# OER-9000/MB-iSTFT-VITS

Hardware: AMD Instinct MI355X
Metric: audio samples/sec (22.05 kHz), MB-iSTFT-VITS infer, batch 64 per GPU (higher is better)
Workload: dtype f32; 1 GPU; configs[1]: ljs_mb_istft_vits, batch 64 per GPU, infer(noise_scale=0, length_scale=1), all 8 outputs; global_batch=64, t_text=200, t_frames_max=566, parallelism=utterance-sharded dp1

## Files before the change

include/mbistft_vits.h:

```cpp
#ifndef MBISTFT_VITS_H
#define MBISTFT_VITS_H

#include <stddef.h>
#include <stdint.h>

#ifdef __cplusplus
extern "C" {
#endif

#define MBV_ABI_VERSION 3

#define MBV_DEC_MULTIBAND   0
#define MBV_DEC_MULTISTREAM 1
#define MBV_DEC_SINGLEBAND  2

typedef struct mbv_model mbv_model;

typedef struct mbv_config {
  int32_t struct_bytes;
  int32_t n_vocab;
  int32_t inter_channels;
  int32_t hidden_channels;
  int32_t filter_channels;
  int32_t n_heads;
// ... 200 lines not shown
  const float *chan_add;
  const float *res;
  const float *res_chan_add;
  const float *accum_in;
  float out_scale;
  const int64_t *trim_lens;
  int32_t trim_num, trim_add;
  int32_t splitk;
  int32_t prec;
  int32_t legacy_convt;
  int64_t ws_floats;
  int32_t n_counters;
  const float *ln_gamma;
  const float *ln_beta;
  const int32_t *ln_out_lens;
} mbv_conv_desc;
#define MBV_ROUTE_NARROW_M 1
#define MBV_ROUTE_NARROW_LAUNCH 2
#define MBV_ROUTE_M64 3
#define MBV_ROUTE_HALF 4
#define MBV_ROUTE_SMALL 5
#define MBV_ROUTE_BIG 6
#define MBV_ROUTE_SPLIT_BATCH 7
#define MBV_ROUTE_VS 8
int mbv_op_conv(mbv_model *m, const mbv_conv_desc *d, const float *x, const float *w_host, const float *bias_host,
                float *y, int32_t *plan_out, void *stream);
int mbv_conv_plan(const mbv_conv_desc *d, int32_t out[8]);

int mbv_op_embed(mbv_model *m, const int64_t *ids, const int64_t *lengths, const float *emb, float *x, int32_t *lens32,
                 int32_t *bad, int B, int T, int H, int n_vocab, void *stream);
int mbv_op_layernorm(mbv_model *m, const float *a, const float *r, const float *gamma, const float *beta, float *y,
                     int B, int C, int T, int pre_relu, const int32_t *out_lens, void *stream);
int mbv_op_durations(mbv_model *m, const float *h, const float *w, const float *bias, const int32_t *lens,
                     float length_scale, float *logw, float *w_ceil, int32_t *cum, int32_t *ylen32, int64_t *ylen64,
                     const int32_t *bad, int B, int C, int T, void *stream);
int mbv_op_expand(mbv_model *m, const float *stats, const int32_t *cum, const int32_t *ylen32, const float *noise,
                  float noise_scale, float *m_p, float *logs_p, float *z_p, float *z, float *attn, float *y_mask,
                  int B, int I, int T, int Tp, void *stream);
int mbv_op_cond_gemv(mbv_model *m, const float *g, const float *W, const float *bias, float *out, int B, int Cin,
                     int Cout, void *stream);
int mbv_op_gather_rows(mbv_model *m, const float *table, const int64_t *sid, float *out, int B, int C, int n_rows,
                       int32_t *bad, void *stream);
// ... 26 lines not shown
```

mb-istft-vits_amd/_capi.py:

```python
import ctypes as C
import os
import subprocess

_HERE = os.path.dirname(os.path.abspath(__file__))
CSRC = os.path.join(_HERE, "csrc")
LIB_PATH = os.environ.get("MBV_LIB") or os.path.join(CSRC, "libmbistft_vits.so")

SYMBOLS = [
    "mbv_abi_version", "mbv_create", "mbv_destroy", "mbv_last_error", "mbv_load_weight",
    "mbv_finalize_weights", "mbv_missing_weights", "mbv_encode", "mbv_synthesize", "mbv_decode",
    "mbv_speaker_embedding", "mbv_stage_times_ms", "mbv_istft_pqmf", "mbv_read_stage",
    "mbv_op_conv1d", "mbv_kernel_times_ms", "mbv_istft_finalize", "mbv_pcm16", "mbv_voice_conversion",
    "mbv_set_option", "mbv_arena_floats", "mbv_export_arena", "mbv_import_arena", "mbv_ticket", "mbv_stage_times_ms_at", "mbv_op_rel_attention",
    "mbv_pcm16_samples", "mbv_resample", "mbv_resample_bank", "mbv_op_conv", "mbv_conv_plan",
    "mbv_spectrogram", "mbv_spectrogram_frames", "mbv_decoder_context", "mbv_decode_range",
    "mbv_resample_ready", "mbv_resample_pcm16_range",
    "mbv_ragged_classes", "mbv_decode_ragged", "mbv_synthesize_ragged", "mbv_ragged_plan",
    "mbv_chunks_plan", "mbv_decode_chunks", "mbv_decoder_runs",
    "mbv_pcm_chunks_plan", "mbv_resample_pcm16_chunks", "mbv_wire_runs",
    "mbv_op_embed", "mbv_op_layernorm", "mbv_op_durations", "mbv_op_expand", "mbv_op_cond_gemv", "mbv_op_gather_rows",
    "mbv_op_posterior_sample", "mbv_op_lens", "mbv_op_dds_sep", "mbv_op_dds_res", "mbv_op_sdp_pre", "mbv_op_sdp_spline",
    "mbv_op_sdp_logw", "mbv_op_sdp_noise", "mbv_op_chan_add",
    "mbv_align", "mbv_set_durations", "mbv_op_neg_cent", "mbv_op_max_path",
    "mbv_admit_plan", "mbv_encode_rows", "mbv_synthesize_rows", "mbv_encoder_runs", "mbv_get_option",
]


ABI_VERSION = 3

# ... 40 lines not shown

class MbvAlignOutputs(C.Structure):
    _fields_ = [(n, C.c_void_p) for n in
                ("w", "attn", "x_mask", "y_mask", "z", "z_p", "m_p", "logs_p", "neg_cent")]


class MbvConvDesc(C.Structure):
    _fields_ = [(n, C.c_int32) for n in ("B", "Cin", "Cout", "Tin", "T", "K", "dil", "x_rstride", "kind", "epi")] + [
        ("in_slope", C.c_float), ("relu", C.c_int32), ("reflect1", C.c_int32),
        ("in_lens", C.c_void_p), ("out_lens", C.c_void_p), ("chan_add", C.c_void_p), ("res", C.c_void_p),
        ("res_chan_add", C.c_void_p), ("accum_in", C.c_void_p), ("out_scale", C.c_float),
        ("trim_lens", C.c_void_p), ("trim_num", C.c_int32), ("trim_add", C.c_int32),
        ("splitk", C.c_int32), ("prec", C.c_int32), ("legacy_convt", C.c_int32),
        ("ws_floats", C.c_int64), ("n_counters", C.c_int32),
        ("ln_gamma", C.c_void_p), ("ln_beta", C.c_void_p), ("ln_out_lens", C.c_void_p),
    ]


CONV_KIND_CONV, CONV_KIND_CONVT4, CONV_KIND_CONVT8 = 0, 4, 8
CONV_EPI_STORE, CONV_EPI_RESID, CONV_EPI_RESID_ACC, CONV_EPI_LN = 0, 1, 2, 7
ROUTES = {1: "NARROW_M", 2: "NARROW_LAUNCH", 3: "M64", 4: "HALF", 5: "SMALL", 6: "BIG", 7: "SPLIT_BATCH", 8: "VS"}
PLAN_FIELDS = ("route", "bm", "bn", "threads", "ck", "nb_big", "vs_tv", "S")


def build(force=False, verbose=False):
    if force:
        for f in os.listdir(CSRC):
            if f.endswith(".o") or f.endswith(".so"):
                os.remove(os.path.join(CSRC, f))
    r = subprocess.run(["bash", os.path.join(CSRC, "build.sh")], capture_output=True, text=True)
# ... 51 lines not shown
    L.mbv_spectrogram_frames.restype = C.c_int64
    L.mbv_set_option.argtypes = [vp, C.c_char_p, i32]
    L.mbv_ticket.argtypes = [vp]
    L.mbv_ticket.restype = C.c_int64
    L.mbv_stage_times_ms_at.argtypes = [vp, C.c_int64, C.POINTER(C.c_float * 5)]
    L.mbv_arena_floats.argtypes = [vp]
    L.mbv_arena_floats.restype = C.c_int64
    L.mbv_export_arena.argtypes = [vp, vp, C.c_int64, vp]
    L.mbv_import_arena.argtypes = [vp, vp, C.c_int64, vp]
    L.mbv_read_stage.argtypes = [vp, C.c_char_p, vp, C.c_int64, vp]
    L.mbv_read_stage.restype = C.c_int64
    L.mbv_op_rel_attention.argtypes = [vp, vp, vp, vp, vp, vp, i32, i32, i32, i32, vp]
    L.mbv_op_conv1d.argtypes = [vp, vp, vp, vp, vp, i32, i32, i32, i32, i32, i32, C.c_float, vp]
    L.mbv_op_conv.argtypes = [vp, C.POINTER(MbvConvDesc), vp, vp, vp, vp, C.POINTER(C.c_int32 * 8), vp]
    L.mbv_conv_plan.argtypes = [C.POINTER(MbvConvDesc), C.POINTER(C.c_int32 * 8)]
    f32 = C.c_float
    L.mbv_op_embed.argtypes = [vp, vp, vp, vp, vp, vp, vp, i32, i32, i32, i32, vp]
    L.mbv_op_layernorm.argtypes = [vp, vp, vp, vp, vp, vp, i32, i32, i32, i32, vp, vp]
    L.mbv_op_durations.argtypes = [vp, vp, vp, vp, vp, f32, vp, vp, vp, vp, vp, vp, i32, i32, i32, vp]
    L.mbv_op_expand.argtypes = [vp, vp, vp, vp, vp, f32, vp, vp, vp, vp, vp, vp, i32, i32, i32, i32, vp]
    L.mbv_op_cond_gemv.argtypes = [vp, vp, vp, vp, vp, i32, i32, i32, vp]
    L.mbv_op_gather_rows.argtypes = [vp, vp, vp, vp, i32, i32, i32, vp, vp]
    L.mbv_op_posterior_sample.argtypes = [vp, vp, vp, vp, vp, i32, i32, i32, vp]
    L.mbv_op_lens.argtypes = [vp, vp, vp, vp, vp, i32, i32, vp]
    L.mbv_op_dds_sep.argtypes = [vp, vp, vp, vp, vp, vp, vp, vp, i32, i32, i32, i32, i32, vp]
    L.mbv_op_dds_res.argtypes = [vp, vp, vp, vp, vp, vp, i32, i32, i32, vp, vp]
    L.mbv_op_sdp_pre.argtypes = [vp, vp, i32, vp, vp, vp, vp, i32, i32, i32, vp]
    L.mbv_op_sdp_spline.argtypes = [vp, vp, vp, vp, i32, i32, i32, f32, vp]
    L.mbv_op_sdp_logw.argtypes = [vp, vp, vp, vp, vp, vp, i32, i32, vp]
    L.mbv_op_sdp_noise.argtypes = [vp, vp, f32, vp, C.c_int64, vp]
# ... 51 lines not shown
```

mb-istft-vits_amd/csrc/capi.hip:

```cpp
#include "../../include/mbistft_vits.h"
#include "kernels.h"

#include <algorithm>
#include <array>
#include <cmath>
#include <cstdarg>
#include <cstdio>
#include <cstdlib>
#include <cstring>
#include <map>
#include <string>
#include <vector>

using namespace mbv;

namespace {

constexpr int kWindow = 4;
constexpr int kDpFilter = 256;
constexpr int kFlowLayers = 4;
constexpr int kFlowK = 5;
constexpr int kNFlows = 4;
constexpr float kLrelu = 0.1f;

// ... 1052 lines not shown
            a.accum_in = j == 0 ? nullptr : xs;
            a.out_scale = j == 2 ? (1.f / 3.f) : 1.f;
          }
          if (rr) a.in_lens = i == 0 ? rr->len_u : rr->len_uu;
          with_trim(a, Lo / Td, 0);
          launch_conv1d(a, s, rt_num * (Lo / Td));
          state = r;
        }
        continue;
      }
      for (int q = 0; q < 3; ++q) {
        const int d = c.resblock_dilations[j][q];
        {
          ConvArgs a = conv_args(m, R.c1[q], state, (int64_t)ch * Lo, Lo, t1, (int64_t)ch * Lo, Lo, B, d);
          a.in_slope = kLrelu;
          if (q == 0) a.chan_add = cadd;
          own_ws(a);
          if (rr) a.in_lens = i == 0 ? rr->len_u : rr->len_uu;
          with_trim(a, Lo / Td, 0);
          launch_conv1d(a, s, rt_num * (Lo / Td));
        }
        {
          ConvArgs a = conv_args(m, R.c2[q], t1, (int64_t)ch * Lo, Lo, r, (int64_t)ch * Lo, Lo, B, 1);
          a.in_slope = kLrelu;
          a.res = state; a.res_bstride = (int64_t)ch * Lo;
          if (q == 0) a.res_chan_add = cadd;
          if (q < 2) {
            a.epi = EPI_RESID;
          } else {
            a.epi = EPI_RESID_ACC;
            a.y = xs;
            a.accum_in = j == 0 ? nullptr : xs;
            a.out_scale = j == 2 ? (1.f / 3.f) : 1.f;
            if (conc && j > 0) HIPCHK(m, hipStreamWaitEvent(s, m->ev_rb[j - 1], 0));
          }
          own_ws(a);
          if (rr) a.in_lens = i == 0 ? rr->len_u : rr->len_uu;
          with_trim(a, Lo / Td, 0);
          launch_conv1d(a, s, rt_num * (Lo / Td));
// ... 2247 lines not shown
  }
  ConvArgs a{};
  a.Tin = d.Tin; a.x_rstride = d.x_rstride ? d.x_rstride : d.Tin; a.Cin = d.Cin;
  a.x_bstride = (int64_t)d.Cin * a.x_rstride;
  a.M = convt ? U * d.Cout : d.Cout;
  a.Mpad = (int)align_up(a.M, 128);
  a.K = convt ? 16 / U + 1 : d.K;
  a.dil = convt ? 1 : d.dil;
  a.pad_left = convt ? (U == 4 ? 2 : 1) : (a.K - 1) * a.dil / 2;
  a.in_slope = d.in_slope;
  a.in_lens = d.in_lens; a.chan_add = d.chan_add; a.reflect1 = d.reflect1;
  a.T = d.T;
  a.y_bstride = (int64_t)d.Cout * d.T * (convt ? U : 1);
  a.epi = convt ? EPI_CONVT : d.epi;
  a.convt_u = convt ? U : 0;
  a.relu = d.relu; a.out_lens = d.out_lens;
  a.res = d.res; a.res_bstride = (int64_t)d.Cout * d.T; a.res_chan_add = d.res_chan_add;
  a.accum_in = d.accum_in; a.out_scale = d.epi == MBV_CONV_EPI_RESID_ACC ? d.out_scale : 1.f;
  a.B = d.B;
  a.splitk = d.splitk != 0;
  a.prec = d.prec;
  if ((a.epi == EPI_RESID || a.epi == EPI_RESID_ACC) && (unsigned long long)a.M * a.T * 4ull >= (1ull << 32))
    return "one utterance's output exceeds 4 GiB";
  if (ln) {
    a.ln_gamma = d.ln_gamma; a.ln_beta = d.ln_beta; a.ln_out_lens = d.ln_out_lens;
    if (!conv1d_narrow_supported(a)) return "LN outside the narrow kernel's range (conv1d_narrow_supported)";
  }
  *out = a;
  return nullptr;
}

// ... 25 lines not shown
int mbv_conv_plan(const mbv_conv_desc* d, int32_t out[8]) {
  if (!d || !out) { g_create_error = "mbv_conv_plan: NULL argument"; return 1; }
  ConvArgs a{};
  const char* why = conv_desc_args(*d, &a);
  ConvPlan p{};
  if (!why) {
    a.ws_floats = d->ws_floats > 0 ? (size_t)d->ws_floats : 0;
    a.n_counters = d->n_counters > 0 ? d->n_counters : 0;
    why = conv_desc_plan(*d, a, &p);
  }
  if (why) { g_create_error = std::string("mbv_conv_plan: ") + why; return 1; }
  plan_ints(p, out);
  return 0;
}

int mbv_op_conv(mbv_model* m, const mbv_conv_desc* d, const float* x, const float* w_host, const float* bias_host,
                float* y, int32_t* plan_out, void* stream) {
  if (!m) return 1;
  if (!d || !x || !w_host || !y) return m->fail("mbv_op_conv: NULL argument");
  ConvArgs a{};
  const char* why = conv_desc_args(*d, &a);
  if (why) return m->fail("mbv_op_conv: %s", why);
  a.ws = m->conv_ws; a.ws_floats = m->conv_ws_floats; a.counters = m->conv_cnt; a.n_counters = m->conv_ncnt;
  if (m->splitk && !d->trim_lens) a.splitk = 1;
  ConvPlan p{};
  if ((why = conv_desc_plan(*d, a, &p))) return m->fail("mbv_op_conv: %s", why);
  DEVICE_GUARD(m);
  hipStream_t s = (hipStream_t)stream;
  DevAllocs mem;
  auto upload = [&](const void* src, size_t bytes, void** dst) -> int {
    HIPCHK(m, hipMalloc(dst, bytes));
    mem.p.push_back(*dst);
    HIPCHK(m, hipMemcpy(*dst, src, bytes, hipMemcpyHostToDevice));
    return 0;
  };
  const bool convt = a.epi == EPI_CONVT;
  const int U = a.convt_u;
// ... 45 lines not shown
```

mb-istft-vits_amd/csrc/conv1d.hip:

```cpp
#include "kernels.h"
#include <cstdio>
#include <cstdlib>

#ifndef MBV_CONV_GLDS
#define MBV_CONV_GLDS 8
#endif
namespace mbv {

typedef float f32x16 __attribute__((ext_vector_type(16)));
typedef float f32x4 __attribute__((ext_vector_type(4)));

__device__ __forceinline__ float lrelu(float v, float slope) { return v > 0.f ? v : v * slope; }
__device__ __forceinline__ float sigmoidf_(float v) { return 1.f / (1.f + expf(-v)); }

#ifdef MBV_CONV_STAMPS
#define MBV_CSTAMP(ID)                                                                        \
  if ((tid & 255) == 0 && stamp_n < 511) stamp_lds[tid >> 8][++stamp_n] = (__builtin_amdgcn_s_memrealtime() << 4) | (unsigned)(ID);
#define MBV_CSTAMP_FLUSH()                                                                    \
  {                                                                                           \
    if ((tid & 255) == 0) stamp_lds[tid >> 8][0] = stamp_n;                                   \
    __syncthreads();                                                                          \
    unsigned long long* sb_ = reinterpret_cast<unsigned long long*>(a.ws) + (size_t)blockIdx.x * 1024; \
    for (int e = tid; e < 1024; e += NT) sb_[e] = stamp_lds[e >> 9][e & 511];                 \
  }
// ... 117 lines not shown
                if (a.accum_in) v0 += a.accum_in[(int64_t)b * a.y_bstride + (int64_t)row * a.T + t];
              } else if constexpr (EPI == EPI_RES_SKIP) {
                if (row < a.split) v0 = a.y[(int64_t)b * a.y_bstride + (int64_t)row * a.T + t];
                else if (a.skip_accum) v0 = a.skip[((int64_t)b * (a.M - a.split) + (row - a.split)) * a.T + t];
              } else {
                v0 = a.couple_sign * a.y[(int64_t)b * a.y_bstride + (int64_t)row * a.T + t];
              }
            }
          }
          acc[i][j][r] = v0;
        }
      }
    }
}

template <int WM, int WN, int CK, int NWN, int EPI, int PREC = 0, int NWM = 2, int VS = 0>
__global__ __launch_bounds__(64 * NWM * NWN, 2) void conv1d_mfma_kernel(const ConvArgs a, int tiles_x,
                                                                        int tiles_y, int total_tiles,
                                                                        int ksplit) {
  constexpr int NT = 64 * NWM * NWN;
  constexpr bool DB = NWN == 4;
  constexpr int BM = 32 * WM * NWM;
  constexpr int BN = 32 * WN * NWN;
  constexpr int G = CK / 8;
  extern __shared__ __attribute__((aligned(16))) float lds[];

  const int tid = threadIdx.x;
  const int lane = tid & 63;
#ifdef MBV_CONV_STAMPS
  int stamp_n = 0;
  __shared__ unsigned long long stamp_lds[2][512];
// ... 5 lines not shown
  const int halo = (a.K - 1) * a.dil;
  const int XL = BN + halo;
  const int buf_f4 = G * 2 * XL + a.K * G * 2 * BM + 2 * BM;
  f32x4* const lds4 = reinterpret_cast<f32x4*>(lds);
  const int tin_eff = a.reflect1 ? a.Tin + 1 : a.Tin;

  constexpr int HALO_MAX = CK == 8 ? 72 : (CK == 16 ? 24 : 0);
  constexpr int KMAX = CK == 8 ? 11 : (CK == 16 ? 5 : 1);
  constexpr int NXP = (G * 2 * (BN + HALO_MAX) + NT - 1) / NT;
  constexpr int NW = (KMAX * G * 2 * BM + NT - 1) / NT;
  constexpr int RPI = NT / BM;
  constexpr int ROWS_PER_TAP = 2 * G;
  static_assert(RPI % ROWS_PER_TAP == 0 || ROWS_PER_TAP % RPI == 0, "weight-row decomposition");
  constexpr bool GLDS = DB && (CK <= MBV_CONV_GLDS || NWM == 1);
  f32x4 wreg[GLDS ? 1 : NW];
  f32x4 xreg[NXP];
  int xoff[NXP];
  const int totalW = a.K * ROWS_PER_TAP * BM;
  const int wq = tid % BM, wR0 = tid / BM;
  const int wtap0 = RPI >= ROWS_PER_TAP ? wR0 / ROWS_PER_TAP : 0;
  const int wrem0 = RPI >= ROWS_PER_TAP ? wR0 % ROWS_PER_TAP : wR0;
  const int64_t tap_stride = (int64_t)(a.Cin / 8) * 2 * a.Mpad * 4;

  int lb = 0, lm0 = 0, lt0 = 0;
  const float* wlane = nullptr;
  const float* xb = nullptr;

#define MBV_SETUP_TILE(TILE)                                                                 \
  {                                                                                          \
    const int tile_ = (TILE);                                                                \
    if (a.trim_map) {                     \
      const int ux_ = tile_ / tiles_y;                                                       \
      lb = a.trim_map[a.B + 1 + ux_]; lm0 = (tile_ % tiles_y) * BM; lt0 = (ux_ - a.trim_map[lb]) * BN; \
    } else {                                                                                 \
      const int tx_ = tile_ % tiles_x, rest_ = tile_ / tiles_x;                              \
      lb = rest_ / tiles_y; lm0 = (rest_ % tiles_y) * BM; lt0 = tx_ * BN;                    \
    }                                                                                        \
    wlane = (PREC == 3 ? a.w_split : a.w) + (int64_t)wtap0 * tap_stride + ((int64_t)wrem0 * a.Mpad + lm0 + wq) * 4; \
    xb = a.x + (int64_t)lb * a.x_bstride;                                                    \
    const int len_in_ = a.in_lens ? a.in_lens[lb] : 0x7fffffff;                              \
    int P = tid / XL, col = tid - P * XL;                                                    \
    _Pragma("unroll") for (int u = 0; u < NXP; ++u) {                                        \
      int off = -1;                                                                          \
      if (P < 2 * G) {                                                                       \
        int gi = lt0 - a.pad_left + col;                                                     \
        if constexpr (VS) {      \
          if (gi >= 0) {                                                                     \
            const int bq_ = gi / a.vs_tv, tq_ = gi - bq_ * a.vs_tv;                          \
            if (bq_ < a.B && tq_ < a.Tin && (!a.in_lens || tq_ < a.in_lens[bq_]))            \
              off = bq_ * (int)a.x_bstride + ((P >> 1) * 8 + (P & 1)) * a.x_rstride + tq_;   \
          }                                                                                  \
        } else                                                                               \
        if (gi >= 0 && gi < tin_eff) {                                                       \
          if (a.reflect1) gi = gi == 0 ? 1 : gi - 1;                                         \
          if (gi < len_in_) off = ((P >> 1) * 8 + (P & 1)) * a.x_rstride + gi;               \
        }                                                                                    \
      }                                                                                      \
      xoff[u] = off;                                                                         \
      col += NT;                                                                             \
      _Pragma("unroll") for (int w = 0; w < NT / 128; ++w)                                   \
        if (col >= XL) { col -= XL; ++P; }                                                   \
    }                                                                                        \
  }
#define MBV_ISSUE(CN)                                                                        \
  {                                                                                          \
    const int cn_ = (CN);                                                                    \
    const float* wchunk = wlane + (int64_t)(cn_ / 8) * 2 * a.Mpad * 4;                       \
    if constexpr (!GLDS) {                                                                   \
    _Pragma("unroll") for (int u = 0; u < NW; ++u) {                                         \
      int64_t off;                                                                           \
      if constexpr (RPI >= ROWS_PER_TAP) {                                                   \
        int tap = wtap0 + u * (RPI / ROWS_PER_TAP);     \
        tap = tap < a.K ? tap : a.K - 1;                                                     \
        off = (int64_t)(tap - wtap0) * tap_stride;                                           \
      } else {                                                                               \
        constexpr int PPT = ROWS_PER_TAP / RPI;                          \
        int tap = u / PPT;                                                 \
        tap = tap < a.K ? tap : a.K - 1;                                                     \
        off = tap * tap_stride + (int64_t)((u % PPT) * RPI) * a.Mpad * 4;                    \
      }                                                                                      \
      wreg[u] = *reinterpret_cast<const f32x4*>(wchunk + off);                               \
    }                                                                                        \
    }                                                                                        \
    const float* xchunk = xb + (int64_t)cn_ * a.x_rstride;                                   \
    const unsigned rs2 = 2u * (unsigned)a.x_rstride;                                         \
    _Pragma("unroll") for (int u = 0; u < NXP; ++u) {                                        \
      f32x4 v = {0.f, 0.f, 0.f, 0.f};                                                        \
      if (xoff[u] >= 0) {                                                                    \
        const unsigned o = (unsigned)xoff[u];                                                \
        v[0] = xchunk[o]; v[1] = xchunk[o + rs2]; v[2] = xchunk[o + 2 * rs2]; v[3] = xchunk[o + 3 * rs2]; \
      }                                                                                      \
      xreg[u] = v;                                                                           \
    }                                                                                        \
  }
#define MBV_COMMIT(CN, XS, WS)                                                               \
  {                                                                                          \
    const int cn_ = (CN);                                                                    \
    if constexpr (!GLDS) {                                                                   \
    _Pragma("unroll") for (int u = 0; u < NW; ++u) {                                         \
      const int e = tid + NT * u;                                                            \
      if (e < totalW) (WS)[e] = wreg[u];                        \
    }                                                                                        \
    }                                                                                        \
    int P = tid / XL, col = tid - P * XL;                                                    \
    _Pragma("unroll") for (int u = 0; u < NXP; ++u) {                                        \
      if (P < 2 * G) {                                                                       \
        f32x4 v = {0.f, 0.f, 0.f, 0.f};                                                      \
        if (xoff[u] >= 0) {                                                                  \
          v = xreg[u];                                                                       \
          if (a.chan_add) {                                                                  \
            const float* ca = a.chan_add + lb * a.Cin + cn_ + (P >> 1) * 8 + (P & 1);        \
            v[0] += ca[0]; v[1] += ca[2]; v[2] += ca[4]; v[3] += ca[6];                      \
          }                                                                                  \
          _Pragma("unroll") for (int s4 = 0; s4 < 4; ++s4) v[s4] = lrelu(v[s4], a.in_slope); \
        }                                                                                    \
        (XS)[P * XL + col] = PREC == 3 ? split_slot(v) : v;                                  \
      }                                                                                      \
      col += NT;                                                                             \
      _Pragma("unroll") for (int w = 0; w < NT / 128; ++w)                                   \
        if (col >= XL) { col -= XL; ++P; }                                                   \
    }                                                                                        \
  }

#define MBV_GLDS_W(CN, WS)                                                                   \
  {                                                                                          \
    const float* wchunk = wlane + (int64_t)((CN) / 8) * 2 * a.Mpad * 4;                      \
    const int wave_e0 = __builtin_amdgcn_readfirstlane(tid & ~63);                           \
    const unsigned lds0 = __builtin_amdgcn_readfirstlane(                                    \
        (unsigned)(size_t)(__attribute__((address_space(3))) void*)((WS) + wave_e0));        \
    _Pragma("unroll") for (int u = 0; u < NW; ++u) {                                         \
      int64_t off;                                                                           \
      if constexpr (RPI >= ROWS_PER_TAP) {                                                   \
        off = (int64_t)(u * (RPI / ROWS_PER_TAP)) * tap_stride;                              \
      } else {                                                                               \
        constexpr int PPT = ROWS_PER_TAP / RPI;                                              \
        off = (u / PPT) * tap_stride + (int64_t)((u % PPT) * RPI) * a.Mpad * 4;              \
      }                                                                                      \
      if (wave_e0 + NT * u < totalW) {                 \
        unsigned keep_m0;                                                                    \
        asm volatile("s_mov_b32 %0, m0\n\ts_mov_b32 m0, %2\n\ts_nop 0\n\t"                  \
                     "global_load_lds_dwordx4 %1, off\n\ts_mov_b32 m0, %0"                   \
                     : "=&s"(keep_m0) : "v"(wchunk + off), "s"(lds0 + (unsigned)(NT * u * 16)) : "memory"); \
      }                                                                                      \
    }                                                                                        \
  }
#define MBV_GLDS_DRAIN() asm volatile("s_waitcnt vmcnt(0)" ::: "memory")

  const int nck = a.Cin / CK;
  const int S = NWN == 2 ? ksplit : 1;
  if (a.trim_map) total_tiles = a.trim_map[a.B] * tiles_y;
  const int total_units = total_tiles * S;
  __shared__ int s_ticket;
  int s_unit = blockIdx.x;
  int s_c = (s_unit % S) * nck / S, s_end = (s_unit % S + 1) * nck / S;
  int pend_cn = -1;
#define MBV_ISSUE_NEXT()                                                                     \
  if (s_unit < total_units) {                                                                \
    const bool first_ = s_c == (s_unit % S) * nck / S;                                       \
    if (first_) MBV_SETUP_TILE(s_unit / S);                                                  \
    MBV_ISSUE(s_c * CK);                                                                     \
    pend_cn = s_c * CK;                                                                      \
    if (++s_c == s_end) {                                                                    \
      s_unit += gridDim.x;                                                                   \
      s_c = (s_unit % S) * nck / S;                                                          \
      s_end = (s_unit % S + 1) * nck / S;                                                    \
    }                                                                                        \
  }

  MBV_ISSUE_NEXT();
  {
    f32x4* const X0 = lds4;
    f32x4* const W0 = X0 + G * 2 * XL;
    if (pend_cn >= 0) {
      if constexpr (GLDS) { MBV_GLDS_W(pend_cn, W0); }
      MBV_COMMIT(pend_cn, X0, W0);
    }
    pend_cn = -1;
  }
  if constexpr (GLDS) { MBV_GLDS_DRAIN(); }
  __syncthreads();

  int q = 0;
  for (int unit = blockIdx.x; unit < total_units; unit += gridDim.x) {
    const int tile = unit / S, sp = unit % S;
    const int c_lo = sp * nck / S, c_hi = (sp + 1) * nck / S;
    int b, m0, t0;
    if (a.trim_map) {
      const int ux = tile / tiles_y;
      b = a.trim_map[a.B + 1 + ux]; m0 = (tile % tiles_y) * BM; t0 = (ux - a.trim_map[b]) * BN;
    } else {
      const int tx = tile % tiles_x, rest = tile / tiles_x;
      b = rest / tiles_y; m0 = (rest % tiles_y) * BM; t0 = tx * BN;
    }
    const int wrow0 = m0 + wm * 32 * WM;
// ... 39 lines not shown
      for (int i = 0; i < WM; ++i)
#pragma unroll
        for (int j = 0; j < WN; ++j) asm volatile("" : "+v"(acc[i][j]));
#endif
    }
    MBV_CSTAMP(2)

    for (int c = c_lo; c < c_hi; ++c, ++q) {
      f32x4* const Xs = lds4 + (DB ? ((q & 1) ? buf_f4 : 0) : 0);
      f32x4* const Ws = Xs + G * 2 * XL;
      f32x4* const Xn = lds4 + (DB ? ((q & 1) ? 0 : buf_f4) : 0);
      f32x4* const Wn = Xn + G * 2 * XL;
      if constexpr (!DB) { MBV_ISSUE_NEXT(); }
      if constexpr (GLDS) {
        if (pend_cn >= 0) { MBV_GLDS_W(pend_cn, Wn); }
      }

      MBV_CSTAMP(3)
      const int nsteps = a.K * G;
      const f32x4* wbase = Ws + hl * BM + wm * 32 * WM + l31;
      const f32x4* xbase = Xs + hl * XL + wn * 32 * WN + l31;
      if (nact == WM || (PREC == 3 && nact > 0)) {
        f32x4 a0[WM], b0[WN], a1[WM], b1[WN];
#define MBV_LOAD_AB(ST, AV, BV)                                                   \
        {                                                                          \
          const int st_ = (ST);                                                    \
          const int tap_ = st_ / G, g_ = st_ % G;                                  \
          const f32x4* wp_ = wbase + st_ * (2 * BM);                               \
          const f32x4* xp_ = xbase + g_ * (2 * XL) + tap_ * a.dil;                 \
          _Pragma("unroll") for (int i = 0; i < WM; ++i) AV[i] = wp_[i * 32];      \
// ... 99 lines not shown
#pragma unroll
          for (int j = 0; j < WN; ++j) {
            const f32x4 bv = xp[j * 32];
#pragma unroll
            for (int s4 = 0; s4 < 4; ++s4)
              acc[0][j] = __builtin_amdgcn_mfma_f32_32x32x2f32(av[s4], bv[s4], acc[0][j], 0, 0, 0);
          }
        }
      }

      MBV_CSTAMP(4)
      if constexpr (DB) {
        if (pend_cn >= 0) { MBV_COMMIT(pend_cn, Xn, Wn); }
        pend_cn = -1;
        MBV_CSTAMP(9)
        if constexpr (GLDS) { MBV_GLDS_DRAIN(); }
        MBV_CSTAMP(10)
        if (c + 1 < c_hi) { MBV_ISSUE_NEXT(); }
        MBV_CSTAMP(5)
        __syncthreads();
        MBV_CSTAMP(6)
      } else {
        if (pend_cn >= 0) {
          __syncthreads();
          MBV_COMMIT(pend_cn, Xn, Wn);
          pend_cn = -1;
          __syncthreads();
        }
      }
    }

// ... 120 lines not shown
          }
        }
      }
    } else if ((EPI == EPI_STORE || EPI == EPI_RESID || EPI == EPI_RESID_ACC) && full && !a.out_lens) {
      float* py = a.y + (int64_t)b * a.y_bstride + lane_off;
#pragma unroll
      for (int i = 0; i < WM; ++i)
#pragma unroll
        for (int r = 0; r < 16; ++r) {
          const int k0 = i * 32 + (r & 3) + 8 * (r >> 2);
          const float bias = __shfl(rowc, k0 + 4 * hl);
          float* q = py + (int64_t)k0 * T;
#pragma unroll
          for (int j = 0; j < WN; ++j) {
            float v = acc[i][j][r] + bias;
            if constexpr (EPI == EPI_STORE) { if (a.relu) v = fmaxf(v, 0.f); }
            if constexpr (EPI == EPI_RESID_ACC) v *= a.out_scale;
            q[j * 32] = v;
          }
        }
    } else if (EPI == EPI_RES_SKIP && full && a.split % 32 == 0) {
      const int64_t col_off = (int64_t)(4 * hl) * T + t0 + wn * 32 * WN + l31;
#pragma unroll
      for (int i = 0; i < WM; ++i) {
        const int trow = wrow0 + i * 32;
        const bool is_x = trow < a.split;
        float* base = is_x ? a.y + (int64_t)b * a.y_bstride + (int64_t)trow * T
                           : a.skip + ((int64_t)b * (a.M - a.split) + (trow - a.split)) * T;
#pragma unroll
        for (int r = 0; r < 16; ++r) {
          const int k0 = (r & 3) + 8 * (r >> 2);
// ... 30 lines not shown
#pragma unroll
        for (int r = 0; r < 16; ++r) {
          const int k = i * 32 + (r & 3) + 8 * (r >> 2) + 4 * hl;
          const float bias = __shfl(rowc, k);
          const int row = wrow0 + k;
          if (i >= nact || row >= a.M) continue;
#pragma unroll
          for (int j = 0; j < WN; ++j) {
            const int t = t0 + wn * 32 * WN + j * 32 + l31;
            if (t >= T) continue;
            float v = acc[i][j][r] + bias;
            const float mask = t < len_out ? 1.f : 0.f;
            const int64_t o = (int64_t)b * a.y_bstride + (int64_t)row * T + t;
            if constexpr (EPI == EPI_STORE) {
              if (a.relu) v = fmaxf(v, 0.f);
              if (a.out_lens) v *= mask;
              a.y[o] = v;
            } else if constexpr (EPI == EPI_RESID) {
              a.y[o] = v;
            } else if constexpr (EPI == EPI_RESID_ACC) {
              a.y[o] = v * a.out_scale;
            } else if constexpr (EPI == EPI_RES_SKIP) {
              if (row < a.split) a.y[o] = v * mask;
              else a.skip[((int64_t)b * (a.M - a.split) + (row - a.split)) * T + t] = v;
            } else if constexpr (EPI == EPI_COUPLE) {
              a.y[o] = a.couple_sign * v * mask;
            }
          }
        }
      }
    }
    MBV_CSTAMP(8)
  }
  MBV_CSTAMP_FLUSH()
#undef MBV_ISSUE_NEXT
#undef MBV_SETUP_TILE
#undef MBV_ISSUE
#undef MBV_COMMIT
#undef MBV_GLDS_W
#undef MBV_GLDS_DRAIN
}

constexpr int kSplitkTinyDiv = 16;
static int conv_splitk_factor(const ConvArgs& a, int BM, int BN, int CK, int NWN, int NT, long total, bool trimmed) {
  const long slots = 256L * (NT == 512 ? 1 : 2);
  int S = 1;
  const int nck = a.Cin / CK;
  const bool tiny = total * (long)kSplitkTinyDiv <= slots;
  const int min_chunks = tiny ? 2 : 4;
  if (NWN == 2 && a.splitk && a.ws_floats && a.n_counters && total * 4 <= slots && nck >= (tiny ? 4 : 16) &&
      total <= a.n_counters && !trimmed) {
    S = (int)(slots / total);
    if (S > nck / min_chunks) S = nck / min_chunks;
    if (S > 16) S = 16;
    while (S > 1 && (size_t)total * S * BM * BN > a.ws_floats) --S;
    if (S < 1) S = 1;
  }
  return S;
}

template <int WM, int WN, int CK, int NWN, int EPI, int PREC = 0, int NWM = 2, int VS = 0>
static void launch_epi(const ConvArgs& a, hipStream_t s) {
  constexpr int BM = 32 * WM * NWM, BN = 32 * WN * NWN, G = CK / 8, NT = 64 * NWM * NWN;
  const int XL = BN + (a.K - 1) * a.dil;
  const size_t buf_f4 = (size_t)G * 2 * XL + (size_t)a.K * G * 2 * BM + 2 * BM;
  const size_t lds_bytes = buf_f4 * 16 * (NWN == 4 ? 2 : 1);
  const int tiles_x = VS ? (int)(((long)a.B * a.vs_tv + BN - 1) / BN) : (a.T + BN - 1) / BN, tiles_y = (a.M + BM - 1) / BM;
  const long total = VS ? (long)tiles_x * tiles_y : (long)tiles_x * tiles_y * a.B;
  const long slots = 256L * (NT == 512 ? 1 : 2);
  const int S = conv_splitk_factor(a, BM, BN, CK, NWN, NT, total, a.trim_map != nullptr);
  if (a.trim_map && a.trim_bn != BN) {
    fprintf(stderr, "mbv: trimmed decode: tile map built for %d-column tiles, the launch uses %d\n", a.trim_bn, BN);
    abort();
  }
  const long units = total * S;
  const int grid = (int)(units > slots ? slots : units);
  static bool attr = false;
  if (!attr) {
    (void)hipFuncSetAttribute(reinterpret_cast<const void*>(&conv1d_mfma_kernel<WM, WN, CK, NWN, EPI, PREC, NWM, VS>),
                              hipFuncAttributeMaxDynamicSharedMemorySize,
#ifdef MBV_CONV_STAMPS
                              150 * 1024);
#else
                              160 * 1024 - 256);
#endif
    attr = true;
  }
  hipLaunchKernelGGL((conv1d_mfma_kernel<WM, WN, CK, NWN, EPI, PREC, NWM, VS>), dim3(grid), dim3(NT), lds_bytes, s, a,
                     tiles_x, tiles_y, (int)total, S);
}

template <int WM, int WN, int CK, int NWN>
static void launch_one(const ConvArgs& a, hipStream_t s) {
  if constexpr (WM == 2) {
    if (a.prec == 3) {
      if constexpr (CK <= 16) {
        switch (a.epi) {
          case EPI_STORE: launch_epi<WM, WN, CK, NWN, EPI_STORE, 3>(a, s); return;
          case EPI_RESID: launch_epi<WM, WN, CK, NWN, EPI_RESID, 3>(a, s); return;
          case EPI_RESID_ACC: launch_epi<WM, WN, CK, NWN, EPI_RESID_ACC, 3>(a, s); return;
          case EPI_CONVT:
            if constexpr (CK == 16) { launch_epi<WM, WN, CK, NWN, EPI_CONVT, 3>(a, s); return; }
            break;
// ... 123 lines not shown
    }
    shape(CONV_M64, 64, 128, 256, ck);
  }
  const long total = (long)((a.T + p.bn - 1) / p.bn) * ((a.M + p.bm - 1) / p.bm) * a.B;
  p.S = conv_splitk_factor(a, p.bm, p.bn, p.ck, p.bn == 384 ? 4 : 2, p.threads, total, trimmed);
  return p;
}

int conv1d_trim_bn(const ConvArgs& a) {
  if (a.epi == EPI_LN || a.splitk) return 0;
  const int r = conv1d_plan(a, false).route;
  if (r == CONV_NARROW_M || r == CONV_NARROW_LAUNCH) return 0;
  return conv1d_plan(a, true).bn;
}

void launch_conv1d(const ConvArgs& a, hipStream_t s, int route_T) {
  if ((a.epi == EPI_RESID || a.epi == EPI_RESID_ACC) && (unsigned long long)a.M * a.T * 4ull >= (1ull << 32)) {
    fprintf(stderr, "mbv: conv1d: one utterance's [%d x %d] output exceeds 4 GiB\n", a.M, a.T);
    abort();
  }
  if (a.epi == EPI_LN && !conv1d_narrow_supported(a)) { fprintf(stderr, "mbv: EPI_LN outside the narrow kernel's range\n"); abort(); }
  const ConvPlan p = conv1d_plan(a, a.trim_map != nullptr, route_T);
  switch (p.route) {
    case CONV_NARROW_M: launch_conv1d_narrow(a, false, s); return;
    case CONV_NARROW_LAUNCH: launch_conv1d_narrow(a, true, s); return;
    case CONV_VS: {
      ConvArgs av = a;
      av.vs_tv = p.vs_tv;
      launch_epi<2, 3, 16, 4, EPI_CONVT, 0, 2, 1>(av, s);
      return;
    }
    case CONV_SPLIT_BATCH: {
      ConvArgs a1 = a, a2 = a;
      const int nb = p.nb_big;
      a1.B = nb;
      a2.B = a.B - nb;
      a2.x += (int64_t)nb * a.x_bstride;
      a2.y += (int64_t)nb * a.y_bstride;
      if (a.in_lens) a2.in_lens += nb;
      if (a.out_lens) a2.out_lens += nb;
      if (a.chan_add) a2.chan_add += (int64_t)nb * a.Cin;
      if (a.res) a2.res += (int64_t)nb * a.res_bstride;
      if (a.res_chan_add) a2.res_chan_add += (int64_t)nb * a.M;
      if (a.accum_in) a2.accum_in += (int64_t)nb * a.y_bstride;
      if (a.gate_cond) a2.gate_cond += (int64_t)nb * a.gate_cond_bstride;
      if (a.skip) a2.skip += (int64_t)nb * (a.M - a.split) * a.T;
      launch_ck<2, 3, 4>(a1, s);
      launch_ck<2, 2, 2>(a2, s);
      return;
    }
    case CONV_BIG: launch_ck<2, 3, 4>(a, s); return;
    case CONV_SMALL: launch_ck<2, 2, 2>(a, s); return;
    case CONV_HALF:
      if (p.ck == 16) {
        switch (a.epi) {
          case EPI_STORE: launch_epi<2, 3, 16, 4, EPI_STORE, 0, 1>(a, s); return;
          case EPI_RESID: launch_epi<2, 3, 16, 4, EPI_RESID, 0, 1>(a, s); return;
          default: launch_epi<2, 3, 16, 4, EPI_RESID_ACC, 0, 1>(a, s); return;
        }
      }
      switch (a.epi) {
        case EPI_STORE: launch_epi<2, 3, 8, 4, EPI_STORE, 0, 1>(a, s); return;
        case EPI_RESID: launch_epi<2, 3, 8, 4, EPI_RESID, 0, 1>(a, s); return;
        default: launch_epi<2, 3, 8, 4, EPI_RESID_ACC, 0, 1>(a, s); return;
      }
    default: launch_ck<1, 2, 2>(a, s); return;
// ... 5 lines not shown
```

mb-istft-vits_amd/csrc/conv1d_narrow.hip:

```cpp
#include "kernels.h"
#include <cstdio>

namespace mbv {

namespace {

typedef float f32x16 __attribute__((ext_vector_type(16)));
typedef float f32x4 __attribute__((ext_vector_type(4)));

constexpr int kHalf = 16;
constexpr int kRsrcFlags = 0x00020000;
constexpr unsigned kOob = 0x7fffffffu;

__device__ __forceinline__ f32x4 bload4(__amdgpu_buffer_rsrc_t r, unsigned voff, unsigned soff) {
  return __builtin_bit_cast(f32x4, __builtin_amdgcn_raw_buffer_load_b128(r, (int)voff, (int)soff, 0));
}
__device__ __forceinline__ float bload1(__amdgpu_buffer_rsrc_t r, unsigned voff, unsigned soff) {
  return __builtin_bit_cast(float, __builtin_amdgcn_raw_buffer_load_b32(r, (int)voff, (int)soff, 0));
}
__device__ __forceinline__ void bstore1(float v, __amdgpu_buffer_rsrc_t r, unsigned voff, unsigned soff) {
  __builtin_amdgcn_raw_buffer_store_b32(__builtin_bit_cast(int, v), r, (int)voff, (int)soff, 0);
}
__device__ __forceinline__ float lrelu_(float v, float slope) { return v > 0.f ? v : v * slope; }

// ... 334 lines not shown
    } else
    {
      const bool keep = !a.out_lens || t < a.out_lens[b];
#pragma unroll
      for (int j = 0; j < NRT; ++j) {
        const int row0 = MBV_ROW0(j);
        if (row0 >= M) continue;
#pragma unroll
        for (int r = 0; r < 16; ++r) {
          const int k = (r & 3) + 8 * (r >> 2);
          float v = acc[j][r];
          if constexpr (kExtra == 1) v += acc2[j][r];
          if constexpr (kExtra == 3) v = (v + acc2[j][r]) + (acc2[NRT + j][r] + acc2[2 * NRT + j][r]);
          if constexpr (EPI == EPI_STORE) {
            if (a.relu) v = fmaxf(v, 0.f);
            if (!keep) v = 0.f;
          } else if constexpr (EPI == EPI_RESID_ACC) {
            v *= a.out_scale;
          }
          if (row0 + k + 4 * hl < M) bstore1(v, y_rs, y_voff, (unsigned)(row0 + k) * rowT);
        }
      }
    }
    MBV_STAMP(5)
#undef MBV_ROW0
  }
#pragma unroll
  for (int i = 0; i < kPF; ++i) asm volatile("" ::"v"(pfv[i]));
}

// ... 82 lines not shown
```

mb-istft-vits_amd/csrc/kernels.h:

```cpp
#pragma once
#include <hip/hip_runtime.h>
#include <stdint.h>

#include <vector>

namespace mbv {

enum ConvEpilogue : int {
  EPI_STORE = 0,
  EPI_RESID = 1,
  EPI_RESID_ACC = 2,
  EPI_GATE = 3,
  EPI_RES_SKIP = 4,
  EPI_COUPLE = 5,
  EPI_CONVT = 6,
  EPI_LN = 7,
};

struct ConvArgs {
  const float* x;
  int64_t x_bstride;
  int Tin;
  int x_rstride;
  int Cin;
// ... 29 lines not shown
  int B;
  const int* trim_map;
  int trim_bn;
  int vs_tv;
  float* ws;
  size_t ws_floats;
  unsigned* counters;
  int n_counters;
  int convt_u;
  int splitk;
  int prec;
  const float* w_split;
  const float* ln_gamma;
  const float* ln_beta;
  const int* ln_out_lens;
};
enum ConvRoute : int {
  CONV_NARROW_M = 1,
  CONV_NARROW_LAUNCH = 2,
  CONV_M64 = 3,
  CONV_HALF = 4,
  CONV_SMALL = 5,
  CONV_BIG = 6,
  CONV_SPLIT_BATCH = 7,
  CONV_VS = 8,
};
struct ConvPlan {
  int route;
  int bm, bn, threads, ck;
  int nb_big;
  int vs_tv;
  int S;
};
ConvPlan conv1d_plan(const ConvArgs& a, bool trimmed, int route_T = 0);
inline ConvPlan conv1d_plan(const ConvArgs& a) { return conv1d_plan(a, a.trim_map != nullptr); }
void launch_conv1d(const ConvArgs& a, hipStream_t s, int route_T = 0);
bool conv1d_supported(int K, int dil);
bool conv1d_narrow_supported(const ConvArgs& a);
void launch_conv1d_narrow(const ConvArgs& a, bool by_launch_size, hipStream_t s);

struct WnLayerArgs {
  const float* h_in;
  float* h_out;
  float* skip;
  const int* lens;
  const int* ustart;
  const int* hmap;
  const float* wg; const float* bg;
  const float* gcond;
  int gcond_bstride;
  const float* wr; const float* br;
// ... 221 lines not shown
```

Measured before the change: 176.2 million samples/s.

## Move ResBlock leaky-relu into conv1 epilogue and DMA input windows to LDS

The first conv of each decoder ResBlock pair now applies leaky-relu in its store epilogue (out_slope), so the second conv reads pre-activated input with in_slope=1. That lets the big MFMA conv route load its input window straight from global memory into LDS with global_load_lds_dword instead of staging it through registers. The aim is to cut register pressure and VALU copy work in the input staging path of the residual convs. The cost is inline asm that manipulates m0, a separate zero-fill path for out-of-range columns, and extra kernel template instantiations.

Result: no change. 175.6 million samples/s (-0.4%).

```diff
diff --git a/include/mbistft_vits.h b/include/mbistft_vits.h
--- a/include/mbistft_vits.h
+++ b/include/mbistft_vits.h
@@ -238,6 +238,7 @@
   const float *ln_gamma;
   const float *ln_beta;
   const int32_t *ln_out_lens;
+  float out_slope;
 } mbv_conv_desc;
 #define MBV_ROUTE_NARROW_M 1
 #define MBV_ROUTE_NARROW_LAUNCH 2
@@ -250,6 +251,7 @@
 int mbv_op_conv(mbv_model *m, const mbv_conv_desc *d, const float *x, const float *w_host, const float *bias_host,
                 float *y, int32_t *plan_out, void *stream);
 int mbv_conv_plan(const mbv_conv_desc *d, int32_t out[8]);
+int mbv_conv_window_dma(const mbv_conv_desc *d, int32_t *out);
 
 int mbv_op_embed(mbv_model *m, const int64_t *ids, const int64_t *lengths, const float *emb, float *x, int32_t *lens32,
                  int32_t *bad, int B, int T, int H, int n_vocab, void *stream);
diff --git a/mb-istft-vits_amd/_capi.py b/mb-istft-vits_amd/_capi.py
--- a/mb-istft-vits_amd/_capi.py
+++ b/mb-istft-vits_amd/_capi.py
@@ -12,7 +12,7 @@
     "mbv_speaker_embedding", "mbv_stage_times_ms", "mbv_istft_pqmf", "mbv_read_stage",
     "mbv_op_conv1d", "mbv_kernel_times_ms", "mbv_istft_finalize", "mbv_pcm16", "mbv_voice_conversion",
     "mbv_set_option", "mbv_arena_floats", "mbv_export_arena", "mbv_import_arena", "mbv_ticket", "mbv_stage_times_ms_at", "mbv_op_rel_attention",
-    "mbv_pcm16_samples", "mbv_resample", "mbv_resample_bank", "mbv_op_conv", "mbv_conv_plan",
+    "mbv_pcm16_samples", "mbv_resample", "mbv_resample_bank", "mbv_op_conv", "mbv_conv_plan", "mbv_conv_window_dma",
     "mbv_spectrogram", "mbv_spectrogram_frames", "mbv_decoder_context", "mbv_decode_range",
     "mbv_resample_ready", "mbv_resample_pcm16_range",
     "mbv_ragged_classes", "mbv_decode_ragged", "mbv_synthesize_ragged", "mbv_ragged_plan",
@@ -83,6 +83,7 @@
         ("splitk", C.c_int32), ("prec", C.c_int32), ("legacy_convt", C.c_int32),
         ("ws_floats", C.c_int64), ("n_counters", C.c_int32),
         ("ln_gamma", C.c_void_p), ("ln_beta", C.c_void_p), ("ln_out_lens", C.c_void_p),
+        ("out_slope", C.c_float),
     ]
 
 
@@ -164,6 +165,7 @@
     L.mbv_op_conv1d.argtypes = [vp, vp, vp, vp, vp, i32, i32, i32, i32, i32, i32, C.c_float, vp]
     L.mbv_op_conv.argtypes = [vp, C.POINTER(MbvConvDesc), vp, vp, vp, vp, C.POINTER(C.c_int32 * 8), vp]
     L.mbv_conv_plan.argtypes = [C.POINTER(MbvConvDesc), C.POINTER(C.c_int32 * 8)]
+    L.mbv_conv_window_dma.argtypes = [C.POINTER(MbvConvDesc), C.POINTER(C.c_int32)]
     f32 = C.c_float
     L.mbv_op_embed.argtypes = [vp, vp, vp, vp, vp, vp, vp, i32, i32, i32, i32, vp]
     L.mbv_op_layernorm.argtypes = [vp, vp, vp, vp, vp, vp, i32, i32, i32, i32, vp, vp]
diff --git a/mb-istft-vits_amd/csrc/capi.hip b/mb-istft-vits_amd/csrc/capi.hip
--- a/mb-istft-vits_amd/csrc/capi.hip
+++ b/mb-istft-vits_amd/csrc/capi.hip
@@ -1090,6 +1090,7 @@
         {
           ConvArgs a = conv_args(m, R.c1[q], state, (int64_t)ch * Lo, Lo, t1, (int64_t)ch * Lo, Lo, B, d);
           a.in_slope = kLrelu;
+          a.out_slope = kLrelu;
           if (q == 0) a.chan_add = cadd;
           own_ws(a);
           if (rr) a.in_lens = i == 0 ? rr->len_u : rr->len_uu;
@@ -1098,7 +1099,7 @@
         }
         {
           ConvArgs a = conv_args(m, R.c2[q], t1, (int64_t)ch * Lo, Lo, r, (int64_t)ch * Lo, Lo, B, 1);
-          a.in_slope = kLrelu;
+          a.in_slope = 1.f;
           a.res = state; a.res_bstride = (int64_t)ch * Lo;
           if (q == 0) a.res_chan_add = cadd;
           if (q < 2) {
@@ -3376,7 +3377,7 @@
   a.y_bstride = (int64_t)d.Cout * d.T * (convt ? U : 1);
   a.epi = convt ? EPI_CONVT : d.epi;
   a.convt_u = convt ? U : 0;
-  a.relu = d.relu; a.out_lens = d.out_lens;
+  a.relu = d.relu; a.out_lens = d.out_lens; a.out_slope = d.out_slope;
   a.res = d.res; a.res_bstride = (int64_t)d.Cout * d.T; a.res_chan_add = d.res_chan_add;
   a.accum_in = d.accum_in; a.out_scale = d.epi == MBV_CONV_EPI_RESID_ACC ? d.out_scale : 1.f;
   a.B = d.B;
@@ -3432,6 +3433,21 @@
   return 0;
 }
 
+int mbv_conv_window_dma(const mbv_conv_desc* d, int32_t* out) {
+  if (!d || !out) { g_create_error = "mbv_conv_window_dma: NULL argument"; return 1; }
+  ConvArgs a{};
+  const char* why = conv_desc_args(*d, &a);
+  ConvPlan p{};
+  if (!why) {
+    a.ws_floats = d->ws_floats > 0 ? (size_t)d->ws_floats : 0;
+    a.n_counters = d->n_counters > 0 ? d->n_counters : 0;
+    why = conv_desc_plan(*d, a, &p);
+  }
+  if (why) { g_create_error = std::string("mbv_conv_window_dma: ") + why; return 1; }
+  *out = conv1d_window_dma(a, p) ? 1 : 0;
+  return 0;
+}
+
 int mbv_op_conv(mbv_model* m, const mbv_conv_desc* d, const float* x, const float* w_host, const float* bias_host,
                 float* y, int32_t* plan_out, void* stream) {
   if (!m) return 1;
@@ -3439,6 +3455,8 @@
   ConvArgs a{};
   const char* why = conv_desc_args(*d, &a);
   if (why) return m->fail("mbv_op_conv: %s", why);
+  if (a.out_slope != 0.f && (a.epi != EPI_STORE || a.relu))
+    return m->fail("mbv_op_conv: out_slope belongs to a conv with a STORE epilogue and no relu");
   a.ws = m->conv_ws; a.ws_floats = m->conv_ws_floats; a.counters = m->conv_cnt; a.n_counters = m->conv_ncnt;
   if (m->splitk && !d->trim_lens) a.splitk = 1;
   ConvPlan p{};
diff --git a/mb-istft-vits_amd/csrc/conv1d.hip b/mb-istft-vits_amd/csrc/conv1d.hip
--- a/mb-istft-vits_amd/csrc/conv1d.hip
+++ b/mb-istft-vits_amd/csrc/conv1d.hip
@@ -4,6 +4,9 @@
 
 #ifndef MBV_CONV_GLDS
 #define MBV_CONV_GLDS 8
+#endif
+#ifndef MBV_CONV_XDMA
+#define MBV_CONV_XDMA 16
 #endif
 namespace mbv {
 
@@ -155,7 +158,7 @@
     }
 }
 
-template <int WM, int WN, int CK, int NWN, int EPI, int PREC = 0, int NWM = 2, int VS = 0>
+template <int WM, int WN, int CK, int NWN, int EPI, int PREC = 0, int NWM = 2, int VS = 0, int XDMA = 0>
 __global__ __launch_bounds__(64 * NWM * NWN, 2) void conv1d_mfma_kernel(const ConvArgs a, int tiles_x,
                                                                         int tiles_y, int total_tiles,
                                                                         int ksplit) {
@@ -191,8 +194,13 @@
   static_assert(RPI % ROWS_PER_TAP == 0 || ROWS_PER_TAP % RPI == 0, "weight-row decomposition");
   constexpr bool GLDS = DB && (CK <= MBV_CONV_GLDS || NWM == 1);
   f32x4 wreg[GLDS ? 1 : NW];
-  f32x4 xreg[NXP];
-  int xoff[NXP];
+  constexpr bool XD = XDMA != 0;
+  static_assert(!XD || (DB && NWM == 2 && PREC == 0 && VS == 0 && (EPI == EPI_RESID || EPI == EPI_RESID_ACC)), "XDMA shape");
+  f32x4 xreg[XD ? 1 : NXP];
+  int xoff[XD ? 1 : NXP];
+  constexpr int NPW = (G * 2 * (BN + HALO_MAX) + 16 * (NT / 64) - 1) / (16 * (NT / 64));
+  int xdo[XD ? NPW : 1];
+  bool xd_inner = false;
   const int totalW = a.K * ROWS_PER_TAP * BM;
   const int wq = tid % BM, wR0 = tid / BM;
   const int wtap0 = RPI >= ROWS_PER_TAP ? wR0 / ROWS_PER_TAP : 0;
@@ -216,6 +224,23 @@
     wlane = (PREC == 3 ? a.w_split : a.w) + (int64_t)wtap0 * tap_stride + ((int64_t)wrem0 * a.Mpad + lm0 + wq) * 4; \
     xb = a.x + (int64_t)lb * a.x_bstride;                                                    \
     const int len_in_ = a.in_lens ? a.in_lens[lb] : 0x7fffffff;                              \
+    if constexpr (XD) {                                                                      \
+      const int g0_ = lt0 - a.pad_left;                                                      \
+      xd_inner = __builtin_amdgcn_readfirstlane((int)(g0_ >= 0 && g0_ + XL <= a.Tin)) != 0;  \
+      const int e_ = 16 * (tid >> 6) + (lane >> 2);                                          \
+      int P = e_ / XL, col = e_ - P * XL;                                                    \
+      _Pragma("unroll") for (int u = 0; u < NPW; ++u) {                                      \
+        int off = -2;                                                                        \
+        if (P < 2 * G) {                                                                     \
+          const int gi = g0_ + col;                                                          \
+          off = -1;                                                                          \
+          if (gi >= 0 && gi < a.Tin) off = (((P >> 1) * 8 + (P & 1) + 2 * (lane & 3)) * a.x_rstride + gi) * 4; \
+        }                                                                                    \
+        xdo[u] = off;                                                                        \
+        col += 16 * (NT / 64);                                   \
+        if (col >= XL) { col -= XL; ++P; }                                                   \
+      }                                                                                      \
+    } else {                                                                                 \
     int P = tid / XL, col = tid - P * XL;                                                    \
     _Pragma("unroll") for (int u = 0; u < NXP; ++u) {                                        \
       int off = -1;                                                                          \
@@ -238,6 +263,7 @@
       _Pragma("unroll") for (int w = 0; w < NT / 128; ++w)                                   \
         if (col >= XL) { col -= XL; ++P; }                                                   \
     }                                                                                        \
+    }                                                                                        \
   }
 #define MBV_ISSUE(CN)                                                                        \
   {                                                                                          \
@@ -259,6 +285,7 @@
       wreg[u] = *reinterpret_cast<const f32x4*>(wchunk + off);                               \
     }                                                                                        \
     }                                                                                        \
+    if constexpr (!XD) {                                                                     \
     const float* xchunk = xb + (int64_t)cn_ * a.x_rstride;                                   \
     const unsigned rs2 = 2u * (unsigned)a.x_rstride;                                         \
     _Pragma("unroll") for (int u = 0; u < NXP; ++u) {                                        \
@@ -269,6 +296,7 @@
       }                                                                                      \
       xreg[u] = v;                                                                           \
     }                                                                                        \
+    }                                                                                        \
   }
 #define MBV_COMMIT(CN, XS, WS)                                                               \
   {                                                                                          \
@@ -279,6 +307,7 @@
       if (e < totalW) (WS)[e] = wreg[u];                        \
     }                                                                                        \
     }                                                                                        \
+    if constexpr (!XD) {                                                                     \
     int P = tid / XL, col = tid - P * XL;                                                    \
     _Pragma("unroll") for (int u = 0; u < NXP; ++u) {                                        \
       if (P < 2 * G) {                                                                       \
@@ -296,6 +325,7 @@
       col += NT;                                                                             \
       _Pragma("unroll") for (int w = 0; w < NT / 128; ++w)                                   \
         if (col >= XL) { col -= XL; ++P; }                                                   \
+    }                                                                                        \
     }                                                                                        \
   }
 
@@ -322,6 +352,31 @@
     }                                                                                        \
   }
 #define MBV_GLDS_DRAIN() asm volatile("s_waitcnt vmcnt(0)" ::: "memory")
+#define MBV_GLDS_X(CN, XS)                                                                   \
+  {                                                                                          \
+    const float* xchunk = xb + (int64_t)(CN) * a.x_rstride;                                  \
+    const int wv_ = __builtin_amdgcn_readfirstlane(tid >> 6);                                \
+    const unsigned ldsx = __builtin_amdgcn_readfirstlane(                                    \
+        (unsigned)(size_t)(__attribute__((address_space(3))) void*)(XS));                    \
+    const int nslot_ = 2 * G * XL;                                                           \
+    _Pragma("unroll") for (int u = 0; u < NPW; ++u) {                                        \
+      const int s0_ = 16 * (wv_ + (NT / 64) * u);                                            \
+      if (s0_ < nslot_) {                                                  \
+        unsigned keep_m0;                                                                    \
+        if (xd_inner && s0_ + 16 <= nslot_) {                                                \
+          asm volatile("s_mov_b32 %0, m0\n\ts_mov_b32 m0, %3\n\ts_nop 0\n\t"                \
+                       "global_load_lds_dword %1, %2\n\ts_mov_b32 m0, %0"                    \
+                       : "=&s"(keep_m0) : "v"(xdo[u]), "s"(xchunk), "s"(ldsx + (unsigned)s0_ * 16u) : "memory"); \
+        } else if (xdo[u] >= 0) {                                                            \
+          asm volatile("s_mov_b32 %0, m0\n\ts_mov_b32 m0, %3\n\ts_nop 0\n\t"                \
+                       "global_load_lds_dword %1, %2\n\ts_mov_b32 m0, %0"                    \
+                       : "=&s"(keep_m0) : "v"(xdo[u]), "s"(xchunk), "s"(ldsx + (unsigned)s0_ * 16u) : "memory"); \
+        } else if (xdo[u] == -1) {                                                           \
+          reinterpret_cast<float*>(XS)[s0_ * 4 + lane] = 0.f;                                \
+        }                                                                                    \
+      }                                                                                      \
+    }                                                                                        \
+  }
 
   const int nck = a.Cin / CK;
   const int S = NWN == 2 ? ksplit : 1;
@@ -350,11 +405,12 @@
     f32x4* const W0 = X0 + G * 2 * XL;
     if (pend_cn >= 0) {
       if constexpr (GLDS) { MBV_GLDS_W(pend_cn, W0); }
+      if constexpr (XD) { MBV_GLDS_X(pend_cn, X0); }
       MBV_COMMIT(pend_cn, X0, W0);
     }
     pend_cn = -1;
   }
-  if constexpr (GLDS) { MBV_GLDS_DRAIN(); }
+  if constexpr (GLDS || XD) { MBV_GLDS_DRAIN(); }
   __syncthreads();
 
   int q = 0;
@@ -424,6 +480,9 @@
       if constexpr (!DB) { MBV_ISSUE_NEXT(); }
       if constexpr (GLDS) {
         if (pend_cn >= 0) { MBV_GLDS_W(pend_cn, Wn); }
+      }
+      if constexpr (XD) {
+        if (pend_cn >= 0) { MBV_GLDS_X(pend_cn, Xn); }
       }
 
       MBV_CSTAMP(3)
@@ -553,7 +612,7 @@
         if (pend_cn >= 0) { MBV_COMMIT(pend_cn, Xn, Wn); }
         pend_cn = -1;
         MBV_CSTAMP(9)
-        if constexpr (GLDS) { MBV_GLDS_DRAIN(); }
+        if constexpr (GLDS || XD) { MBV_GLDS_DRAIN(); }
         MBV_CSTAMP(10)
         if (c + 1 < c_hi) { MBV_ISSUE_NEXT(); }
         MBV_CSTAMP(5)
@@ -704,7 +763,10 @@
 #pragma unroll
           for (int j = 0; j < WN; ++j) {
             float v = acc[i][j][r] + bias;
-            if constexpr (EPI == EPI_STORE) { if (a.relu) v = fmaxf(v, 0.f); }
+            if constexpr (EPI == EPI_STORE) {
+              if (a.relu) v = fmaxf(v, 0.f);
+              if (a.out_slope != 0.f) v = lrelu(v, a.out_slope);
+            }
             if constexpr (EPI == EPI_RESID_ACC) v *= a.out_scale;
             q[j * 32] = v;
           }
@@ -765,6 +827,7 @@
             const int64_t o = (int64_t)b * a.y_bstride + (int64_t)row * T + t;
             if constexpr (EPI == EPI_STORE) {
               if (a.relu) v = fmaxf(v, 0.f);
+              if (a.out_slope != 0.f) v = lrelu(v, a.out_slope);
               if (a.out_lens) v *= mask;
               a.y[o] = v;
             } else if constexpr (EPI == EPI_RESID) {
@@ -789,6 +852,7 @@
 #undef MBV_ISSUE
 #undef MBV_COMMIT
 #undef MBV_GLDS_W
+#undef MBV_GLDS_X
 #undef MBV_GLDS_DRAIN
 }
 
@@ -810,7 +874,7 @@
   return S;
 }
 
-template <int WM, int WN, int CK, int NWN, int EPI, int PREC = 0, int NWM = 2, int VS = 0>
+template <int WM, int WN, int CK, int NWN, int EPI, int PREC = 0, int NWM = 2, int VS = 0, int XDMA = 0>
 static void launch_epi(const ConvArgs& a, hipStream_t s) {
   constexpr int BM = 32 * WM * NWM, BN = 32 * WN * NWN, G = CK / 8, NT = 64 * NWM * NWN;
   const int XL = BN + (a.K - 1) * a.dil;
@@ -828,7 +892,7 @@
   const int grid = (int)(units > slots ? slots : units);
   static bool attr = false;
   if (!attr) {
-    (void)hipFuncSetAttribute(reinterpret_cast<const void*>(&conv1d_mfma_kernel<WM, WN, CK, NWN, EPI, PREC, NWM, VS>),
+    (void)hipFuncSetAttribute(reinterpret_cast<const void*>(&conv1d_mfma_kernel<WM, WN, CK, NWN, EPI, PREC, NWM, VS, XDMA>),
                               hipFuncAttributeMaxDynamicSharedMemorySize,
 #ifdef MBV_CONV_STAMPS
                               150 * 1024);
@@ -837,7 +901,7 @@
 #endif
     attr = true;
   }
-  hipLaunchKernelGGL((conv1d_mfma_kernel<WM, WN, CK, NWN, EPI, PREC, NWM, VS>), dim3(grid), dim3(NT), lds_bytes, s, a,
+  hipLaunchKernelGGL((conv1d_mfma_kernel<WM, WN, CK, NWN, EPI, PREC, NWM, VS, XDMA>), dim3(grid), dim3(NT), lds_bytes, s, a,
                      tiles_x, tiles_y, (int)total, S);
 }
 
@@ -991,7 +1055,29 @@
   return conv1d_plan(a, true).bn;
 }
 
+bool conv1d_window_dma(const ConvArgs& a, const ConvPlan& p) {
+  if (p.route != CONV_BIG && p.route != CONV_SPLIT_BATCH) return false;
+  if (a.epi != EPI_RESID && a.epi != EPI_RESID_ACC) return false;
+  if (a.in_slope != 1.f || a.prec != 0 || a.chan_add || a.in_lens || a.reflect1) return false;
+  if (p.ck != 8 && p.ck != 16) return false;
+  if (p.ck > MBV_CONV_XDMA) return false;
+  return (int64_t)a.x_rstride * 16 * 4 < (1ll << 31);
+}
+static void launch_big_xdma(const ConvArgs& a, int ck, hipStream_t s) {
+  if (ck == 8) {
+    if (a.epi == EPI_RESID) launch_epi<2, 3, 8, 4, EPI_RESID, 0, 2, 0, 1>(a, s);
+    else launch_epi<2, 3, 8, 4, EPI_RESID_ACC, 0, 2, 0, 1>(a, s);
+  } else {
+    if (a.epi == EPI_RESID) launch_epi<2, 3, 16, 4, EPI_RESID, 0, 2, 0, 1>(a, s);
+    else launch_epi<2, 3, 16, 4, EPI_RESID_ACC, 0, 2, 0, 1>(a, s);
+  }
+}
+
 void launch_conv1d(const ConvArgs& a, hipStream_t s, int route_T) {
+  if (a.out_slope != 0.f && (a.epi != EPI_STORE || a.relu)) {
+    fprintf(stderr, "mbv: conv1d: out_slope belongs to a STORE epilogue without relu\n");
+    abort();
+  }
   if ((a.epi == EPI_RESID || a.epi == EPI_RESID_ACC) && (unsigned long long)a.M * a.T * 4ull >= (1ull << 32)) {
     fprintf(stderr, "mbv: conv1d: one utterance's [%d x %d] output exceeds 4 GiB\n", a.M, a.T);
     abort();
@@ -1022,11 +1108,15 @@
       if (a.accum_in) a2.accum_in += (int64_t)nb * a.y_bstride;
       if (a.gate_cond) a2.gate_cond += (int64_t)nb * a.gate_cond_bstride;
       if (a.skip) a2.skip += (int64_t)nb * (a.M - a.split) * a.T;
-      launch_ck<2, 3, 4>(a1, s);
+      if (conv1d_window_dma(a, p)) launch_big_xdma(a1, p.ck, s);
+      else launch_ck<2, 3, 4>(a1, s);
       launch_ck<2, 2, 2>(a2, s);
       return;
     }
-    case CONV_BIG: launch_ck<2, 3, 4>(a, s); return;
+    case CONV_BIG:
+      if (conv1d_window_dma(a, p)) launch_big_xdma(a, p.ck, s);
+      else launch_ck<2, 3, 4>(a, s);
+      return;
     case CONV_SMALL: launch_ck<2, 2, 2>(a, s); return;
     case CONV_HALF:
       if (p.ck == 16) {
diff --git a/mb-istft-vits_amd/csrc/conv1d_narrow.hip b/mb-istft-vits_amd/csrc/conv1d_narrow.hip
--- a/mb-istft-vits_amd/csrc/conv1d_narrow.hip
+++ b/mb-istft-vits_amd/csrc/conv1d_narrow.hip
@@ -372,6 +372,7 @@
           if constexpr (kExtra == 3) v = (v + acc2[j][r]) + (acc2[NRT + j][r] + acc2[2 * NRT + j][r]);
           if constexpr (EPI == EPI_STORE) {
             if (a.relu) v = fmaxf(v, 0.f);
+            if (a.out_slope != 0.f) v = lrelu_(v, a.out_slope);
             if (!keep) v = 0.f;
           } else if constexpr (EPI == EPI_RESID_ACC) {
             v *= a.out_scale;
diff --git a/mb-istft-vits_amd/csrc/kernels.h b/mb-istft-vits_amd/csrc/kernels.h
--- a/mb-istft-vits_amd/csrc/kernels.h
+++ b/mb-istft-vits_amd/csrc/kernels.h
@@ -67,6 +67,7 @@
   const float* ln_gamma;
   const float* ln_beta;
   const int* ln_out_lens;
+  float out_slope;
 };
 enum ConvRoute : int {
   CONV_NARROW_M = 1,
@@ -88,6 +89,7 @@
 ConvPlan conv1d_plan(const ConvArgs& a, bool trimmed, int route_T = 0);
 inline ConvPlan conv1d_plan(const ConvArgs& a) { return conv1d_plan(a, a.trim_map != nullptr); }
 void launch_conv1d(const ConvArgs& a, hipStream_t s, int route_T = 0);
+bool conv1d_window_dma(const ConvArgs& a, const ConvPlan& p);
 bool conv1d_supported(int K, int dil);
 bool conv1d_narrow_supported(const ConvArgs& a);
 void launch_conv1d_narrow(const ConvArgs& a, bool by_launch_size, hipStream_t s);
```
